# soedinglab/BaMMmotif2

Hardware: AMD Instinct MI355X
Metric: EM seq-positions/sec (and iterations/sec), 1Mx200bp k=2 W=20 (higher is better)
Workload: dtype f32

## Files before the change

### bammmotif2_amd/__init__.py

```python
from . import abi, synth
from .em import (EM, Comm, Context, PackedSeqs, SeqSet, calculate_p, logodds, occurrences, Occurrences, FdrMops, fdr_geometry, seed_from_pwm, sample_negatives, libc_srand,
                 v_size, v_offset, bg_size, bg_offset, device_count, device_pci_bus_id, device_can_access_peer, peer_access_matrix, device_blocks_live, mask_plan)

__all__ = ["EM", "Comm", "Context", "PackedSeqs", "SeqSet", "calculate_p", "logodds", "occurrences", "Occurrences", "FdrMops", "fdr_geometry", "seed_from_pwm", "sample_negatives", "libc_srand",
           "v_size", "v_offset", "bg_size", "bg_offset", "device_count", "device_pci_bus_id", "device_can_access_peer", "peer_access_matrix", "device_blocks_live", "mask_plan", "abi", "synth"]
```

### bammmotif2_amd/abi.py

```python
from __future__ import annotations

import ctypes as C
import os

import numpy as np

HERE = os.path.dirname(os.path.abspath(__file__))
LIB_PATH = os.path.join(HERE, "libbamm_em.so")

OK, ERR_ARG, ERR_HIP, ERR_NO_DEVICE, ERR_UNSUPPORTED, ERR_STATE, ERR_COMM = 0, -1, -2, -3, -4, -5, -6
MAX_ORDER = 10


class BammError(RuntimeError):
    def __init__(self, code: int, msg: str):
        super().__init__(f"bamm error {code}: {msg}")
        self.code = code


class Packed(C.Structure):
    _fields_ = [("n_seqs", C.c_uint64), ("n_words", C.c_uint64), ("n_exc", C.c_uint64),
                ("total_len", C.c_uint64), ("max_len", C.c_uint32), ("min_len", C.c_uint32),
                ("words", C.POINTER(C.c_uint32)), ("word_off", C.POINTER(C.c_uint64)),
                ("len", C.POINTER(C.c_uint32)), ("exc_off", C.POINTER(C.c_uint64)),
# ... 7 lines not shown
                ("n_seqs_global", C.c_uint64), ("n_seqs_bound", C.c_uint64)]


ALLREDUCE_FN = C.CFUNCTYPE(C.c_int, C.c_void_p, C.c_void_p, C.c_uint64, C.c_void_p)

SYMBOLS = [
    "bamm_last_error", "bamm_version", "bamm_pack_kmers", "bamm_pack_kmer_ptrs", "bamm_pack_codes", "bamm_pack_codes_seeded",
    "bamm_unpack_y", "bamm_packed_free", "bamm_shard_range", "bamm_ctx_create", "bamm_ctx_destroy",
    "bamm_ctx_sync", "bamm_ctx_device_name", "bamm_ctx_set_launch", "bamm_ctx_set_tuning", "bamm_seqs_upload",
    "bamm_seqs_destroy", "bamm_seqs_info", "bamm_em_default_params", "bamm_em_create",
    "bamm_em_destroy", "bamm_em_estep", "bamm_em_mstep", "bamm_em_optimize_q", "bamm_em_iterate",
    "bamm_em_optimize", "bamm_em_mask", "bamm_em_accumulate", "bamm_em_reduce_buffer", "bamm_em_update", "bamm_em_set_reduce_buffer",
    "bamm_em_set_allreduce", "bamm_em_set_comm", "bamm_comm_init_all", "bamm_comm_unique_id", "bamm_comm_init_rank",
    "bamm_comm_info", "bamm_comm_destroy", "bamm_comm_time_allreduce", "bamm_em_comm_mode", "bamm_seqs_from_codes", "bamm_seqs_bg_model", "bamm_sample_negatives", "bamm_rand_stream_draws", "bamm_comm_init_local", "bamm_comm_init_shm", "bamm_comm_abort", "bamm_device_count", "bamm_device_pci_bus_id", "bamm_device_can_access_peer", "bamm_em_get_v", "bamm_em_get_counts", "bamm_em_get_s", "bamm_em_get_q",
    "bamm_em_get_llh", "bamm_em_get_vdiff", "bamm_em_get_iteration", "bamm_em_get_r",
    "bamm_em_get_trace", "bamm_em_kernel_time", "bamm_em_set_kernel_timing", "bamm_em_plan", "bamm_em_plan_mixed", "bamm_em_plan_paths", "bamm_mask_plan", "bamm_device_blocks_live", "bamm_seed_from_pwm", "bamm_set_host_threads", "bamm_logodds", "bamm_logodds_subset", "bamm_occurrences", "bamm_occ_info", "bamm_occ_get", "bamm_occ_destroy", "bamm_em_sites", "bamm_sites_info", "bamm_sites_get", "bamm_sites_best", "bamm_sites_destroy", "bamm_fdr_create", "bamm_fdr_add_set", "bamm_fdr_add_scores", "bamm_fdr_seal", "bamm_fdr_absorb", "bamm_fdr_statistics", "bamm_fdr_info", "bamm_fdr_rows", "bamm_fdr_pvalues", "bamm_fdr_geometry", "bamm_fdr_destroy", "bamm_bg_model", "bamm_calculate_p", "bamm_v_size",
    "bamm_v_offset", "bamm_bg_size",
]

_lib = None


def load() -> C.CDLL:
    global _lib
    if _lib is not None:
        return _lib
    if not os.path.exists(LIB_PATH):
        raise ImportError(
            f"{LIB_PATH} is missing: build it with `python -m bammmotif2_amd.build` "
            "(hipcc --offload-arch=gfx950). There is no CPU fallback.")
    L = C.CDLL(LIB_PATH)
# ... 53 lines not shown
    L.bamm_device_pci_bus_id.argtypes = [i, C.c_char_p, C.c_size_t]
    L.bamm_device_can_access_peer.argtypes = [i, i, P(i)]
    for name in ("bamm_em_get_v", "bamm_em_get_counts", "bamm_em_get_s"):
        getattr(L, name).argtypes = [vp, f32p]
    for name in ("bamm_em_get_q", "bamm_em_get_llh", "bamm_em_get_vdiff"):
        getattr(L, name).argtypes = [vp, P(f)]
    L.bamm_em_get_iteration.argtypes = [vp, P(u32)]
    L.bamm_em_get_r.argtypes = [vp, u64, u64, f32p, u64]
    L.bamm_em_get_trace.argtypes = [vp, f32p, f32p, f32p, u32, P(u32)]
    L.bamm_em_kernel_time.argtypes = [vp, P(f), P(u32)]
    L.bamm_em_set_kernel_timing.argtypes = [vp, u32]
    L.bamm_em_plan.argtypes = [vp, P(u64), P(u64), P(u32)]
    L.bamm_em_plan_mixed.argtypes = [vp, P(u64)]
    L.bamm_em_plan_paths.argtypes = [vp, P(i), P(i), P(u64)]
    L.bamm_mask_plan.argtypes = [u32, u32, u32, u64, u64, i, u64p]
    L.bamm_device_blocks_live.argtypes = []
    L.bamm_device_blocks_live.restype = C.c_longlong
    L.bamm_set_host_threads.argtypes = [u32]
    L.bamm_set_host_threads.restype = None
    L.bamm_seed_from_pwm.argtypes = [vp, vp, u32, u32, f32p, f, vp, vp, vp]
    L.bamm_logodds.argtypes = [vp, vp, u32, u32, u32, f32p, f32p, vp, u64, f32p, u64p]
    L.bamm_logodds_subset.argtypes = [vp, vp, vp, u32, u32, u32, f32p, f32p, vp, u64, f32p, u64p]
    L.bamm_occurrences.argtypes = [vp, vp, vp, u32, u32, u32, f32p, f32p, f, P(vp)]
    L.bamm_occ_info.argtypes = [vp, P(u64), P(u64), P(u32), P(f), P(f), P(u64)]
    L.bamm_occ_get.argtypes = [vp, vp, vp, vp, vp, vp, vp, u64]
    L.bamm_occ_destroy.argtypes = [vp]
    L.bamm_em_sites.argtypes = [vp, u64, u64, f, P(vp)]
    L.bamm_sites_info.argtypes = [vp, P(u64), P(u64)]
    L.bamm_sites_get.argtypes = [vp, vp, vp, vp, u64]
    L.bamm_sites_best.argtypes = [vp, vp, vp, vp, u64]
# ... 27 lines not shown
```

### bammmotif2_amd/csrc/common.h

```cpp
#pragma once
#include <hip/hip_runtime.h>

#include <cstdint>
#include <cstdio>
#include <cstring>
#include <map>
#include <memory>
#include <string>
#include <vector>

#include "../../include/bamm_em.h"

namespace bamm {

void set_error(const char* fmt, ...);

#define BAMM_HIP(expr)                                                                        \
    do {                                                                                      \
        hipError_t e_ = (expr);                                                               \
        if (e_ != hipSuccess) {                                                               \
            ::bamm::set_error("%s failed: %s (%s:%d)", #expr, hipGetErrorString(e_), __FILE__, \
                              __LINE__);                                                      \
            return BAMM_ERR_HIP;                                                              \
        }                                                                                     \
// ... 161 lines not shown
    UpdateArgs upd;
    PeerArgs peer;
};

bool grp_geometry(uint32_t K, uint32_t W, uint32_t G, int M, uint32_t waves, bool accum, uint32_t logC, uint32_t layout,
                  GrpGeom* out);
bool grp_plan(uint32_t K, uint32_t W, int M, uint32_t waves, bool many_exceptions, bool enough_work, uint32_t forced_G,
              int forced_layout, uint32_t* G, uint32_t* logC, uint32_t* layout);
bool grp_supported_class(int M, uint32_t K);
int launch_em_grp_long(int mclass, bool accum, bool write_r, const GrpKernelArgs& a, uint32_t blocks, uint32_t threads,
                       hipStream_t st);
int launch_em_grp_xl(int mclass, bool accum, bool write_r, const GrpKernelArgs& a, uint32_t blocks, uint32_t threads,
                     hipStream_t st);
uint32_t grp_max_threads(int M);
bool mix_geometry(uint32_t K, uint32_t W, int M, uint32_t waves, bool accum, GrpGeom* out);
int launch_em_mix(int mclass, bool accum, bool write_r, const GrpKernelArgs& a, uint32_t blocks, uint32_t threads, hipStream_t st);
int launch_em_mix1(int mclass, bool accum, bool write_r, const GrpKernelArgs& a, uint32_t blocks, uint32_t threads, hipStream_t st);
int launch_em_grp(int mclass, bool accum, bool write_r, const GrpKernelArgs& a, uint32_t blocks, uint32_t threads,
                  hipStream_t st);
int launch_mix_records(int mclass, const SeqView& sv, const uint4* xrec, uint32_t W, uint32_t T, uint32_t B, uint2* out,
                       uint32_t num_cus, hipStream_t st);

struct SeedKernelArgs {
    SeqView  sv;
    uint32_t K, W, Y;
    uint32_t max_len, vsize;
    uint32_t table_bytes, count_bytes, wave_bytes;
    const float* score;
    float    q;
    const double* u;
    int*     counts;
    uint32_t* z_out;
    unsigned char* wave_scratch;
};
size_t seed_global_scratch_bytes(const SeedKernelArgs& a, uint32_t num_cus);
// ... 161 lines not shown
```

### bammmotif2_amd/csrc/lane_records.h

```cpp
#pragma once
#include "grouped_kernel.h"

namespace bamm {
namespace {

constexpr uint32_t kMixBj = 6u, kMixNe = 3u, kMixBv = kMixBj + kMixNe;
constexpr uint32_t kMixFixBit = 1u << 31;

template <int M>
__device__ __forceinline__ uint2 mix_lane_record(const RawSeqG<M>& cur, int lane, uint32_t W, uint32_t T, uint32_t B) {
    constexpr uint32_t Y = 64u;
    const uint32_t L = __builtin_amdgcn_readfirstlane(cur.L);
    const uint32_t LW1 = L - W + 1u;
    const uint32_t p0 = (uint32_t)lane * M;

    uint32_t X, sE;
    {
        constexpr int NSEL = RawSeqG<M>::NSEL;
        const uint32_t wi0 = p0 >> 4;
        const uint32_t pE = LW1 - 1u, lpE = pE / (uint32_t)M;
        const uint32_t pe = p0 + (uint32_t)(M - 1);
        const uint32_t sel = (pe >> 4) - wi0;
        uint32_t lo = cur.w[1], hi = cur.w[0];
#pragma unroll
        for (int c = 1; c < NSEL; c++) {
            lo = (sel == (uint32_t)c) ? cur.w[c + 1] : lo;
            hi = (sel == (uint32_t)c) ? cur.w[c] : hi;
        }
        X = __builtin_amdgcn_alignbit(hi, lo, 30u - 2u * (pe & 15u));
        sE = (uint32_t)__builtin_amdgcn_readlane((int)X, (int)lpE) >> (2u * ((uint32_t)(M - 1) - (pE - lpE * (uint32_t)M)));
    }

    const uint32_t lane_b = (uint32_t)lane / T, lane_t = (uint32_t)lane - lane_b * T;
    const uint32_t lane_G = lane_t >= B ? 4u : 3u;
    const uint32_t xw = __builtin_amdgcn_readfirstlane(cur.xr.x);
    const uint32_t Bx = (xw >> 12) & 0xfu;
    const uint32_t xlo = xw & 0xfffu;
    const uint32_t nE = min(kMixNe, L - LW1);
    uint32_t yfix = Y | (Y << 7) | (Y << 14) | (Y << 21);
    const bool fixJ = lane_b < Bx;
    const bool fixE = lane_b >= kMixBj && lane_b < kMixBj + nE;
    if (fixJ || fixE) {
        const uint32_t pv = fixJ ? xlo + lane_b : LW1 + (lane_b - kMixBj);
        const uint32_t xfields = xrec_fields<7>(cur.xr.y, cur.xr.z, cur.xr.w, lane_b + 4u - lane_G);
#pragma unroll
        for (int c = 0; c < 4; c++) {
            uint32_t yc = Y;
            if ((uint32_t)c < lane_G) {
                const uint32_t pos = pv - (lane_G - 1u) + (uint32_t)c;
                if (fixJ) {
                    yc = (xfields >> (7u * (uint32_t)c)) & 0x7fu;
                } else {
                    yc = (sE >> (2u * ((LW1 - 1u - pos) & 15u))) & (Y - 1u);
                }
                if (pos >= LW1) yc = Y;
            }
            yfix = (yfix & ~(0x7fu << (7 * c))) | (yc << (7 * c));
        }
        yfix |= kMixFixBit;
    }
    return make_uint2(X, yfix);
}

struct MixSeq {
    uint32_t seq, L, xw;
    uint2 rec;
    bool ok;
};

__device__ __forceinline__ MixSeq fetch_mix_seq(const SeqView& sv, const uint4* xrec, const uint2* lane_rec, uint32_t t, int lane) {
    MixSeq r;
    r.rec = lane_rec[(size_t)t * 64u + (uint32_t)lane];
    r.seq = pick_sequence(sv, t);
    r.ok = !(sv.mask && !sv.mask[r.seq]);
    r.L = sv.len[r.seq];
// ... 7 lines not shown
```

### bammmotif2_amd/csrc/lane_records.hip

```cpp
#include <algorithm>

#include "lane_records.h"

namespace bamm {
namespace {

constexpr uint32_t kRecThreads = 256u, kRecWaves = kRecThreads / 64u;

template <int M>
__global__ void __launch_bounds__(kRecThreads) k_mix_records(SeqView sv, const uint4* xrec, uint32_t W, uint32_t T, uint32_t B, uint2* out) {
    const int lane = threadIdx.x & 63;
    const uint32_t total_waves = gridDim.x * kRecWaves;
    for (uint32_t t = blockIdx.x * kRecWaves + (threadIdx.x >> 6); t < sv.count; t += total_waves) {
        const RawSeqG<M> cur = fetch_seq_g<M>(sv, xrec, t, lane);
        out[(size_t)t * 64u + (uint32_t)lane] = mix_lane_record<M>(cur, lane, W, T, B);
    }
}

template <int M>
int launch_records(const SeqView& sv, const uint4* xrec, uint32_t W, uint32_t T, uint32_t B, uint2* out, uint32_t blocks, hipStream_t st) {
    return launch_kernel(&k_mix_records<M>, blocks, kRecThreads, 0, st, sv, xrec, W, T, B, out);
}

}

int launch_mix_records(int mclass, const SeqView& sv, const uint4* xrec, uint32_t W, uint32_t T, uint32_t B, uint2* out,
                       uint32_t num_cus, hipStream_t st) {
    if (sv.count == 0u && num_cus != kPrimeOnly) return BAMM_OK;
    const uint32_t blocks = num_cus == kPrimeOnly ? kPrimeOnly
                                                  : std::min((sv.count + kRecWaves - 1u) / kRecWaves, std::max(1u, num_cus) * 8u);
    int rc = BAMM_ERR_UNSUPPORTED;
    switch (mclass) {
        case 3: rc = launch_records<4>(sv, xrec, W, T, B, out, blocks, st); break;
        case 4: rc = launch_records<5>(sv, xrec, W, T, B, out, blocks, st); break;
        case 5: rc = launch_records<6>(sv, xrec, W, T, B, out, blocks, st); break;
        case 6: rc = launch_records<7>(sv, xrec, W, T, B, out, blocks, st); break;
        case 7: rc = launch_records<8>(sv, xrec, W, T, B, out, blocks, st); break;
        case 8: rc = launch_records<10>(sv, xrec, W, T, B, out, blocks, st); break;
        default: set_error("no mixed-row kernel for M class %d", mclass);
    }
    if (rc) return rc;
    if (blocks != kPrimeOnly) BAMM_HIP(hipGetLastError());
    return BAMM_OK;
}

}
```

### bammmotif2_amd/csrc/mixed_kernel.h

```cpp
#pragma once
#include "lane_records.h"

namespace bamm {
namespace {

template <int OFF>
__device__ __forceinline__ void lds_add_u64_exec_big(uint32_t byte_addr, unsigned long long v, unsigned long long mask) {
    static_assert(OFF >= 0 && OFF < 65536, "ds offset field");
    lds_add_u64_exec<OFF>(byte_addr, v, mask);
}

template <int M, int A, int NQ, bool ACCUM, bool WRITE_R, int THREADS>
__global__ void __launch_bounds__(THREADS) k_em_mix(GrpKernelArgs ga) {
    static_assert(M >= 4 && 2 * (M - 1) + 12 <= 32, "a wide group within one lane's run, rows out of one stream window");
    static_assert(A == 1 || A == 2, "wide groups");
    constexpr uint32_t WAVES = THREADS / 64, V = WAVES * kMixBv;
    constexpr uint32_t R5N = 1024u, R5V0 = R5N + 1u, R5T = R5V0 + V;
    constexpr uint32_t R6N = 4096u, R6V0 = R6N + 1u, R6T = R6V0 + V;
    constexpr uint32_t Y = 64u, Ys = 65u;
    if (ga.e.stop != nullptr && *ga.e.stop != 0u) return;
    extern __shared__ __align__(16) unsigned char lds_raw[];
    BAMM_PHASE(0);
    const EmKernelArgs& a = ga.e;
    const GrpGeom& g = ga.g;
    const uint32_t W = a.W, T = g.T, B = g.mixB;
    const uint32_t pad = 4u * NQ - B;
    const uint32_t rs5 = g.rowstride;
    float* sg5 = reinterpret_cast<float*>(lds_raw + g.off_sg);
    float* sg6 = reinterpret_cast<float*>(lds_raw + g.off_sg6);
    const float* s1_stage = reinterpret_cast<const float*>(lds_raw + g.off_s1);
    double* stat_lds = reinterpret_cast<double*>(lds_raw + g.off_stat);
    unsigned long long* cnt5 = reinterpret_cast<unsigned long long*>(lds_raw + g.off_ng);
    unsigned long long* cnt6 = reinterpret_cast<unsigned long long*>(lds_raw + g.off_ng6);
    unsigned long long* n1 = reinterpret_cast<unsigned long long*>(lds_raw + g.off_n1);
    unsigned long long* n1p = reinterpret_cast<unsigned long long*>(lds_raw + g.off_wave);
    const uint32_t n1c = ACCUM ? g.wave_bytes / (Y * 8u) : 0u;

    const int lane = threadIdx.x & 63;
    const uint32_t wave = __builtin_amdgcn_readfirstlane(threadIdx.x >> 6);
    const uint32_t total_waves = gridDim.x * WAVES;
    uint32_t t = blockIdx.x * WAVES + wave;
    MixSeq nxt{};
    if (t < a.sv.count) nxt = fetch_mix_seq(a.sv, ga.xrec, ga.lane_rec, t, lane);

    [[maybe_unused]] float q_fused = 0.0f;
    {
        float* s1w = reinterpret_cast<float*>(lds_raw + g.off_s1);
        const float* s1 = s1_stage;
        bool staged = false;
        if constexpr (ACCUM) {
            if (ga.fused) {
// ... 42 lines not shown
            __syncthreads();
        }
    }

    BAMM_PHASE(2);
    if constexpr (ACCUM) {
        const __attribute__((address_space(4))) GrpKernelArgs* kq =
            (const __attribute__((address_space(4))) GrpKernelArgs*)__builtin_amdgcn_kernarg_segment_ptr();
        asm volatile("" : "+s"(kq));
        if (kq->peer.world > 1u && *kq->peer.err != 0u) return;
    }
    const float q = (ACCUM && ga.fused) ? q_fused : *a.q;
    const float one_minus_q = 1.0f - q;
    const uint32_t lane_b = (uint32_t)lane / T, lane_t = (uint32_t)lane - lane_b * T;
    const bool lane_wide = lane_t >= B;
    const uint32_t lane_col0 = lane_wide ? 3u * B + 4u * (lane_t - B) : 3u * lane_t;
    const uint32_t vbase5 = R5V0 + wave * kMixBv, vbase6 = R6V0 + wave * kMixBv;
    const uint32_t sg5_base = lds_offset(sg5), sg6_base = lds_offset(sg6);

    uint32_t resident_fill = 0u;
#pragma unroll
    for (int c = 0; c < 4; c++)
        if (lane_col0 + (uint32_t)c < n1c) resident_fill |= Y << (7 * c);
    double llh_acc = 0.0, sumr_acc = 0.0;
    uint32_t seq_cnt = 0, last_LW1 = 0;
    float pos_i = 0.0f;
    float pos_m[M];
    constexpr bool kCacheSpec = M <= 7 || THREADS < 1024;
    [[maybe_unused]] int spec[kCacheSpec ? M : 1];
    [[maybe_unused]] uint32_t spec_LW1 = 0, spec_xw = 0xffffffffu;
#pragma unroll
    for (int m = 0; m < M; m++) pos_m[m] = 0.0f;
#pragma unroll
    for (int m = 0; m < (kCacheSpec ? M : 1); m++) spec[m] = -1;
    [[maybe_unused]] GrpLogEntry* my_log = nullptr;
    [[maybe_unused]] uint32_t nlog = 0;
    if constexpr (ACCUM)
        my_log = reinterpret_cast<GrpLogEntry*>(ga.fix_log) + (size_t)(blockIdx.x * WAVES + wave) * ga.fix_log_cap;

    for (; t < a.sv.count; t += total_waves) {
        const MixSeq cur = nxt;
        const __attribute__((address_space(4))) GrpKernelArgs* kp =
            (const __attribute__((address_space(4))) GrpKernelArgs*)__builtin_amdgcn_kernarg_segment_ptr();
        asm volatile("" : "+s"(kp));
        if (t + total_waves < a.sv.count) {
            SeqView sv2;
            sv2.words = nullptr; sv2.word_off = nullptr; sv2.len = kp->e.sv.len; sv2.pos_off = nullptr;
            sv2.exc_off = nullptr; sv2.exc = nullptr; sv2.mask = kp->e.sv.mask; sv2.idx = kp->e.sv.idx; sv2.count = a.sv.count;
            nxt = fetch_mix_seq(sv2, kp->xrec, kp->lane_rec, t + total_waves, lane);
        }
        const uint32_t seq = cur.seq;
        if (WRITE_R && (seq < a.seq_begin || seq >= a.seq_end)) continue;
        if (!cur.ok) continue;
        __builtin_amdgcn_s_setprio(0);
        const uint32_t L = __builtin_amdgcn_readfirstlane(cur.L);
        const uint32_t LW1 = L - W + 1u;
        const uint32_t p0 = (uint32_t)lane * M;

        const uint32_t X = cur.rec.x, yfix = cur.rec.y;
        const bool fix = (int)yfix < 0;
        const uint32_t xw = __builtin_amdgcn_readfirstlane(cur.xw);
        const uint32_t Bx = (xw >> 12) & 0xfu;
        const uint32_t xlo = xw & 0xfffu;
        const uint32_t nE = min(kMixNe, L - LW1);
        float fs[4] = {1.0f, 1.0f, 1.0f, 1.0f};
        const float* const sfix_now = (ACCUM && kp->fused) ? kp->s_block + (size_t)blockIdx.x * (W * Ys) : kp->e.s;
        if (fix) {
#pragma unroll
            for (int c = 0; c < 4; c++) {
                const uint32_t colc = min(lane_col0 + (uint32_t)c, W - 1u);
                fs[c] = sfix_now[__umul24(colc, Ys) + ((yfix >> (7 * c)) & 0x7fu)];
            }
        }
        auto slot_offsets = [&](int (&o)[M]) {
#pragma unroll
            for (int m = 0; m < M; m++) {
                const uint32_t k2 = p0 + m - xlo, k3 = p0 + m - LW1;
                o[m] = (p0 + m < LW1) ? -1 : 0;
                if (k2 < Bx) o[m] = (int)(1u + wave * kMixBv + k2);
                if (k3 < nE) o[m] = (int)(1u + wave * kMixBv + kMixBj + k3);
            }
        };
        uint32_t row5[M], row6[M];
        if constexpr (kCacheSpec) {
            if (LW1 != spec_LW1 || xw != spec_xw) {
                spec_LW1 = LW1; spec_xw = xw;
                slot_offsets(spec);
            }
#pragma unroll
            for (int m = 0; m < M; m++) {
                const bool stream = spec[m] < 0;
                row5[m] = stream ? ((X >> (2 * (M - 1 - m))) & 1023u) : R5N + (uint32_t)spec[m];
                row6[m] = stream ? ((X >> (2 * (M - 1 - m))) & 4095u) : R6N + (uint32_t)spec[m];
            }
        } else {
            int o[M];
            slot_offsets(o);
#pragma unroll
            for (int m = 0; m < M; m++) {
                const bool stream = o[m] < 0;
                row5[m] = stream ? ((X >> (2 * (M - 1 - m))) & 1023u) : R5N + (uint32_t)o[m];
                row6[m] = stream ? ((X >> (2 * (M - 1 - m))) & 4095u) : R6N + (uint32_t)o[m];
            }
        }
        if (fix) {
            const float f = ((fs[0] * fs[1]) * fs[2]) * fs[3];
            if (lane_wide) sg6[(vbase6 + lane_b) * A + (lane_t - B)] = f;
            else sg5[__umul24(vbase5 + lane_b, rs5) + pad + lane_t] = f;
        }
        wave_lds_sync();

        __builtin_amdgcn_s_setprio(2);
        float U[M];
        {
            uint32_t ra[M];
#pragma unroll
            for (int m = 0; m < M; m++) ra[m] = sg5_base + __umul24(row5[m], rs5 * 4u);
            float2 pr[M];
#pragma unroll
            for (int m = 0; m < M; m++) {
#ifdef BAMM_PLAIN_LDS
                if constexpr (A == 2) pr[m] = lds_load<float2>(sg6_base + row6[m] * 8u);
                else pr[m].x = lds_load<float>(sg6_base + row6[m] * 4u);
#else
                if constexpr (A == 2) asm volatile("ds_read_b64 %0, %1" : "=v"(pr[m]) : "v"(sg6_base + row6[m] * 8u));
                else asm volatile("ds_read_b32 %0, %1" : "=v"(pr[m].x) : "v"(sg6_base + row6[m] * 4u));
#endif
            }
            grp_chain<M, 3, NQ>(ra, U);
            lds_wait(pr);
            float w0[M];
#pragma unroll
// ... 39 lines not shown
                const uint32_t p = p0 + m;
                if (p < L) ro[L - 1u - p] = U[m];
            }
        }

        if (ACCUM) {
            __builtin_amdgcn_s_setprio(3);
            unsigned long long F[M], nz[M];
            uint32_t rad6[M], rad5[M];
            const uint32_t c5 = lds_offset(cnt5), c6 = lds_offset(cnt6);
#pragma unroll
            for (int m = 0; m < M; m++) {
                F[m] = to_fixed40_pre(U[m]);
                nz[m] = __ballot(F[m] != 0ull);
                rad6[m] = c6 + row6[m] * 8u;
                rad5[m] = c5 + row5[m] * 8u;
            }
            static_for<A>([&](auto wc) {
                constexpr int w = decltype(wc)::value;
                constexpr int off = (4 * w) % M;
#pragma unroll
                for (int m = 0; m < M; m++)
                    lds_add_u64_exec_big<(int)(w * R6T * 8u)>(rad6[m], F[(m + off) % M], nz[(m + off) % M]);
#pragma unroll
                for (int c = 0; c < 4; c++) {
                    const int idx = (c + off) % M;
                    F[idx] = wave_shl1_u64(F[idx]);
                    nz[idx] >>= 1;
                }
            });
            static_for<4 * NQ>([&](auto uc) {
// ... 7 lines not shown
                    for (int c = 0; c < 3; c++) {
                        const int idx = (c + off) % M;
                        F[idx] = wave_shl1_u64(F[idx]);
                        nz[idx] >>= 1;
                    }
                }
            });
            wave_lds_sync();
            unsigned long long acc = 0ull;
            if (fix) {
                unsigned long long* cell = lane_wide ? cnt6 + (size_t)(T - 1u - lane_t) * R6T + vbase6 + lane_b
                                                     : cnt5 + (size_t)(B - 1u - lane_t) * R5T + vbase5 + lane_b;
                acc = *cell;
                *cell = 0ull;
            }
            if (acc != 0ull) {
#pragma unroll
                for (int c = 0; c < 4; c++) {
                    const uint32_t yc = (yfix >> (7 * c)) & 0x7fu;
                    if (yc < Y && ((resident_fill >> (7 * c + 6)) & 1u) != 0u)
                        atomicAdd(&n1p[(lane_col0 + (uint32_t)c) * Y + yc], acc);
                }
            }
            const uint32_t ylog = yfix | resident_fill;
            const uint32_t code = lane_t | (ylog << 3);
            if ((~ylog & (Y | (Y << 7) | (Y << 14) | (Y << 21))) == 0u) acc = 0ull;
            const unsigned long long nzm = __ballot(acc != 0ull);
            if (acc != 0ull) {
                const uint32_t rank = __builtin_amdgcn_mbcnt_hi((uint32_t)(nzm >> 32), __builtin_amdgcn_mbcnt_lo((uint32_t)nzm, 0u));
                GrpLogEntry* const log_now = reinterpret_cast<GrpLogEntry*>(kp->fix_log) + (size_t)(blockIdx.x * WAVES + wave) * kp->fix_log_cap;
                grp_log_store(log_now, nlog + rank, acc, code);
            }
            nlog += (uint32_t)__builtin_popcountll(nzm);
            wave_lds_sync();
        }
    }

    lds_drain();
    BAMM_PHASE(3);
    __syncthreads();
    BAMM_PHASE(4);
    if (lane == 0) {
        stat_lds[wave * 3 + 0] = llh_acc;
// ... 131 lines not shown
```

### bammmotif2_amd/csrc/plan.cpp

```cpp

#include <atomic>
#include <cmath>

#include "handles.h"

namespace bamm {

namespace {

constexpr size_t kLds = 160 * 1024;

int prime_bucket(bamm_ctx* c, const bamm_em_params& prm, uint32_t Y, bool sliced, const EmBucket& eb) {
    if (hipSetDevice(c->device) != hipSuccess) { set_error("hipSetDevice failed"); return BAMM_ERR_HIP; }
    EmKernelArgs a{};
    a.K = prm.K; a.W = prm.W; a.Y = Y;
    if (eb.mclass == kLongClass) return launch_long_em(a, true, false, false, kPrimeOnly, c->stream);
    const uint32_t threads = bucket_threads(c, eb);
    if (sliced || !eb.grouped) {
        a.logC = 0;
        return launch_em_seq(eb.mclass, false, false, a, kPrimeOnly, threads, c->stream);
    }
    GrpKernelArgs ga{};
    ga.e = a;
    if (!grp_geometry(prm.K, prm.W, eb.G, kMClasses[eb.mclass], threads / 64u, true, eb.logc, eb.layout, &ga.g)) return BAMM_OK;
    if (eb.layout & 8u)
        if (int rc = launch_mix_records(eb.mclass, SeqView{}, nullptr, prm.W, ga.g.T, ga.g.mixB, nullptr, kPrimeOnly, c->stream)) return rc;
    return launch_em_grp(eb.mclass, true, false, ga, kPrimeOnly, threads, c->stream);
}

}

uint32_t default_threads(const bamm_ctx* c, int mclass) {
    uint32_t t = c->threads ? c->threads : max_threads_for_mclass(mclass);
    return std::min(t, max_threads_for_mclass(mclass));
}

uint32_t bucket_threads(const bamm_ctx* c, const EmBucket& b) {
    if (b.mclass == kLongClass) return 256u;
    const uint32_t t = default_threads(c, b.mclass);
    return b.grouped ? std::min(t, grp_max_threads(kMClasses[b.mclass])) : t;
}
// ... 103 lines not shown
                    (capable(n) ? yes : no).push_back(n);
                }
            EmBucket eb;
            eb.mclass = b.mclass; eb.grouped = true; eb.logc = glogc; eb.G = gG; eb.layout = glayout; eb.d_xrec = xr->d_xrec;
            if (all) { eb.count = b.count; eb.d_idx = b.d_idx; }
            else {
                uint32_t* d = nullptr;
                if ((rc = em->mem.upload(&d, yes.data(), yes.size()))) return rc;
                own_lists = true;
                eb.count = (uint32_t)yes.size(); eb.d_idx = d;
            }
            if ((glayout & 8u) && eb.count) {
                uint2* rec = nullptr;
                if ((rc = em->mem.scratch(&rec, (size_t)eb.count * 64u))) return rc;
                if ((rc = launch_mix_records(eb.mclass, make_view(seqs, em->exc, eb.d_idx, eb.count, nullptr), xr->d_xrec, prm->W,
                                             gg.T, gg.mixB, rec, (uint32_t)std::max(1, c->num_cus), st))) return rc;
                eb.d_lane_rec = rec;
            }
            eb.work = (double)eb.count * Mcls * 0.6;
            if (eb.count) em->ebuckets.push_back(eb);
            if (all) continue;
        }
        EmBucket eb;
        eb.mclass = b.mclass;
        if (!no.empty()) {
            uint32_t* d = nullptr;
            if ((rc = em->mem.upload(&d, no.data(), no.size()))) return rc;
            own_lists = true;
            eb.count = (uint32_t)no.size(); eb.d_idx = d;
        } else { eb.count = b.count; eb.d_idx = b.d_idx; }
        eb.work = (double)eb.count * Mcls;
// ... 116 lines not shown
```

### bammmotif2_amd/em.py

```python
from __future__ import annotations

import ctypes as C
from typing import Callable, Optional

import numpy as np

from . import abi
from .abi import check


def _f32(a):
    return np.ascontiguousarray(a, dtype=np.float32)


def _u64(a):
    return np.ascontiguousarray(a, dtype=np.uint64)


def v_size(K: int, W: int) -> int:
    return W * ((4 ** (K + 2) - 4) // 3)


def v_offset(k: int, W: int) -> int:
    return W * ((4 ** (k + 1) - 4) // 3)
# ... 110 lines not shown
    return int(n.value)


def device_blocks_live() -> int:
    return int(abi.load().bamm_device_blocks_live())


MASK_PLAN_FIELDS = ("direct", "wave_global", "wave_bytes", "s_in_lds", "e_table", "m_cols", "m_table", "init_table", "e_waves",
                    "m_waves", "cus", "mblocks", "wave_scratch_bytes")


def mask_plan(W: int, Y: int, max_len: int, n_seqs: int, cells: int, num_cus: int) -> dict:
    out = np.zeros(len(MASK_PLAN_FIELDS), np.uint64)
    check(abi.load().bamm_mask_plan(W, Y, max_len, n_seqs, cells, num_cus, out))
    return dict(zip(MASK_PLAN_FIELDS, (int(x) for x in out)))


def device_pci_bus_id(device: int) -> str:
    buf = C.create_string_buffer(32)
    check(abi.load().bamm_device_pci_bus_id(int(device), buf, 32))
    return buf.value.decode()


def device_can_access_peer(device: int, peer: int) -> bool:
    can = C.c_int(0)
    check(abi.load().bamm_device_can_access_peer(int(device), int(peer), C.byref(can)))
    return bool(can.value)


def peer_access_matrix():
# ... 478 lines not shown
```

### include/bamm_em.h

```cpp
#ifndef BAMM_EM_H_
#define BAMM_EM_H_

#include <stddef.h>
#include <stdint.h>

#ifdef __cplusplus
extern "C" {
#endif

#define BAMM_OK              0
#define BAMM_ERR_ARG        -1
#define BAMM_ERR_HIP        -2
#define BAMM_ERR_NO_DEVICE  -3
#define BAMM_ERR_UNSUPPORTED -4
#define BAMM_ERR_STATE      -5
#define BAMM_ERR_COMM       -6

#define BAMM_MAX_ORDER      10
#define BAMM_MAX_SEQ_POSITIONS 8192u

typedef struct bamm_ctx  bamm_ctx;
typedef struct bamm_seqs bamm_seqs;
typedef struct bamm_em   bamm_em;
typedef struct bamm_comm bamm_comm;
// ... 108 lines not shown
typedef struct bamm_sites bamm_sites;
int  bamm_em_sites(bamm_em* em, uint64_t begin, uint64_t end, float cutoff, bamm_sites** out);
int  bamm_sites_info(const bamm_sites* s, uint64_t* n_sites, uint64_t* n_seqs);
int  bamm_sites_get(const bamm_sites* s, uint64_t* seq, uint32_t* pos, float* r, uint64_t cap);
int  bamm_sites_best(const bamm_sites* s, uint32_t* z, float* r_best, uint32_t* count, uint64_t cap);
int  bamm_sites_destroy(bamm_sites* s);
int  bamm_em_get_trace(bamm_em* em, float* llh, float* v_diff, float* q, uint32_t cap, uint32_t* n);
#define BAMM_TIMING_WHOLE_CALL 0xffffffffu
int  bamm_em_kernel_time(bamm_em* em, float* total_ms, uint32_t* launches);
int  bamm_em_set_kernel_timing(bamm_em* em, uint32_t every);
int  bamm_em_plan(bamm_em* em, uint64_t* grouped_seqs, uint64_t* percolumn_seqs, uint32_t* launches);
int  bamm_em_plan_mixed(bamm_em* em, uint64_t* mixed_seqs);
int  bamm_em_plan_paths(bamm_em* em, int* sliced, int* e_fused, uint64_t* long_seqs);
int  bamm_mask_plan(uint32_t W, uint32_t Y, uint32_t max_len, uint64_t n_seqs, uint64_t cells, int num_cus, uint64_t* out);

int  bamm_seed_from_pwm(bamm_ctx* ctx, bamm_seqs* seqs, uint32_t K, uint32_t W, const float* score,
                        float q, const double* u, int32_t* counts, uint32_t* z);

int  bamm_logodds(bamm_ctx* ctx, bamm_seqs* seqs, uint32_t K, uint32_t W, uint32_t bg_order,
                  const float* v_flat, const float* vbg, float* mops, uint64_t mops_cap,
                  float* zoops, uint64_t* z);

int  bamm_logodds_subset(bamm_ctx* ctx, bamm_seqs* seqs, const uint8_t* seq_mask, uint32_t K, uint32_t W,
                         uint32_t bg_order, const float* v_flat, const float* vbg, float* mops,
                         uint64_t mops_cap, float* zoops, uint64_t* z);

typedef struct bamm_occ bamm_occ;
int  bamm_occurrences(bamm_ctx* ctx, bamm_seqs* positives, bamm_seqs* negatives, uint32_t K, uint32_t W,
                      uint32_t bg_order, const float* v_flat, const float* vbg, float p_cutoff, bamm_occ** out);
int  bamm_occ_info(const bamm_occ* occ, uint64_t* n_hits, uint64_t* n_neg_scores, uint32_t* n_top, float* s_ntop,
// ... 38 lines not shown
```

Measured before the change: 501.9 billion.

## Precompute mixed-row fix-lane log decision and simplify inner-loop row/address math

Moves the per-lane decision of whether a fix lane must log to the global fix log into the precomputed lane record, stored as a bit in the yfix word, and encodes the fix flag in bit 31 of the window word. In the mixed E-step kernel it replaces the per-sequence resident-fill loop and atomics with precomputed ballot masks and exec-masked LDS adds. It also biases row5 offsets so row5/row6 come from a max() instead of selects, and hoists fix addresses. This trims scalar/vector ALU work in the hot loop, at the cost of more subtle encoding invariants. Host-callable test hooks are added for the layout and fix word.

```diff
diff --git a/bammmotif2_amd/__init__.py b/bammmotif2_amd/__init__.py
--- a/bammmotif2_amd/__init__.py
+++ b/bammmotif2_amd/__init__.py
@@ -1,6 +1,6 @@
 from . import abi, synth
 from .em import (EM, Comm, Context, PackedSeqs, SeqSet, calculate_p, logodds, occurrences, Occurrences, FdrMops, fdr_geometry, seed_from_pwm, sample_negatives, libc_srand,
-                 v_size, v_offset, bg_size, bg_offset, device_count, device_pci_bus_id, device_can_access_peer, peer_access_matrix, device_blocks_live, mask_plan)
+                 v_size, v_offset, bg_size, bg_offset, device_count, device_pci_bus_id, device_can_access_peer, peer_access_matrix, device_blocks_live, mask_plan, mix_layout, mix_fix_word)
 
 __all__ = ["EM", "Comm", "Context", "PackedSeqs", "SeqSet", "calculate_p", "logodds", "occurrences", "Occurrences", "FdrMops", "fdr_geometry", "seed_from_pwm", "sample_negatives", "libc_srand",
-           "v_size", "v_offset", "bg_size", "bg_offset", "device_count", "device_pci_bus_id", "device_can_access_peer", "peer_access_matrix", "device_blocks_live", "mask_plan", "abi", "synth"]
+           "v_size", "v_offset", "bg_size", "bg_offset", "device_count", "device_pci_bus_id", "device_can_access_peer", "peer_access_matrix", "device_blocks_live", "mask_plan", "mix_layout", "mix_fix_word", "abi", "synth"]
diff --git a/bammmotif2_amd/abi.py b/bammmotif2_amd/abi.py
--- a/bammmotif2_amd/abi.py
+++ b/bammmotif2_amd/abi.py
@@ -45,7 +45,7 @@
     "bamm_em_set_allreduce", "bamm_em_set_comm", "bamm_comm_init_all", "bamm_comm_unique_id", "bamm_comm_init_rank",
     "bamm_comm_info", "bamm_comm_destroy", "bamm_comm_time_allreduce", "bamm_em_comm_mode", "bamm_seqs_from_codes", "bamm_seqs_bg_model", "bamm_sample_negatives", "bamm_rand_stream_draws", "bamm_comm_init_local", "bamm_comm_init_shm", "bamm_comm_abort", "bamm_device_count", "bamm_device_pci_bus_id", "bamm_device_can_access_peer", "bamm_em_get_v", "bamm_em_get_counts", "bamm_em_get_s", "bamm_em_get_q",
     "bamm_em_get_llh", "bamm_em_get_vdiff", "bamm_em_get_iteration", "bamm_em_get_r",
-    "bamm_em_get_trace", "bamm_em_kernel_time", "bamm_em_set_kernel_timing", "bamm_em_plan", "bamm_em_plan_mixed", "bamm_em_plan_paths", "bamm_mask_plan", "bamm_device_blocks_live", "bamm_seed_from_pwm", "bamm_set_host_threads", "bamm_logodds", "bamm_logodds_subset", "bamm_occurrences", "bamm_occ_info", "bamm_occ_get", "bamm_occ_destroy", "bamm_em_sites", "bamm_sites_info", "bamm_sites_get", "bamm_sites_best", "bamm_sites_destroy", "bamm_fdr_create", "bamm_fdr_add_set", "bamm_fdr_add_scores", "bamm_fdr_seal", "bamm_fdr_absorb", "bamm_fdr_statistics", "bamm_fdr_info", "bamm_fdr_rows", "bamm_fdr_pvalues", "bamm_fdr_geometry", "bamm_fdr_destroy", "bamm_bg_model", "bamm_calculate_p", "bamm_v_size",
+    "bamm_em_get_trace", "bamm_em_kernel_time", "bamm_em_set_kernel_timing", "bamm_em_plan", "bamm_em_plan_mixed", "bamm_em_plan_paths", "bamm_mask_plan", "bamm_mix_layout", "bamm_mix_fix_word", "bamm_device_blocks_live", "bamm_seed_from_pwm", "bamm_set_host_threads", "bamm_logodds", "bamm_logodds_subset", "bamm_occurrences", "bamm_occ_info", "bamm_occ_get", "bamm_occ_destroy", "bamm_em_sites", "bamm_sites_info", "bamm_sites_get", "bamm_sites_best", "bamm_sites_destroy", "bamm_fdr_create", "bamm_fdr_add_set", "bamm_fdr_add_scores", "bamm_fdr_seal", "bamm_fdr_absorb", "bamm_fdr_statistics", "bamm_fdr_info", "bamm_fdr_rows", "bamm_fdr_pvalues", "bamm_fdr_geometry", "bamm_fdr_destroy", "bamm_bg_model", "bamm_calculate_p", "bamm_v_size",
     "bamm_v_offset", "bamm_bg_size",
 ]
 
@@ -129,6 +129,8 @@
     L.bamm_em_plan_mixed.argtypes = [vp, P(u64)]
     L.bamm_em_plan_paths.argtypes = [vp, P(i), P(i), P(u64)]
     L.bamm_mask_plan.argtypes = [u32, u32, u32, u64, u64, i, u64p]
+    L.bamm_mix_layout.argtypes = [u32, i, P(u32)]
+    L.bamm_mix_fix_word.argtypes = [u32, u32, u32, u32, u32, u32, u32, u32, u32, P(u32)]
     L.bamm_device_blocks_live.argtypes = []
     L.bamm_device_blocks_live.restype = C.c_longlong
     L.bamm_set_host_threads.argtypes = [u32]
diff --git a/bammmotif2_amd/csrc/common.h b/bammmotif2_amd/csrc/common.h
--- a/bammmotif2_amd/csrc/common.h
+++ b/bammmotif2_amd/csrc/common.h
@@ -199,11 +199,12 @@
                      hipStream_t st);
 uint32_t grp_max_threads(int M);
 bool mix_geometry(uint32_t K, uint32_t W, int M, uint32_t waves, bool accum, GrpGeom* out);
+inline __host__ __device__ uint32_t mix_resident_cols(const GrpGeom& g) { return g.wave_bytes / (64u * 8u); }
 int launch_em_mix(int mclass, bool accum, bool write_r, const GrpKernelArgs& a, uint32_t blocks, uint32_t threads, hipStream_t st);
 int launch_em_mix1(int mclass, bool accum, bool write_r, const GrpKernelArgs& a, uint32_t blocks, uint32_t threads, hipStream_t st);
 int launch_em_grp(int mclass, bool accum, bool write_r, const GrpKernelArgs& a, uint32_t blocks, uint32_t threads,
                   hipStream_t st);
-int launch_mix_records(int mclass, const SeqView& sv, const uint4* xrec, uint32_t W, uint32_t T, uint32_t B, uint2* out,
+int launch_mix_records(int mclass, const SeqView& sv, const uint4* xrec, uint32_t W, uint32_t T, uint32_t B, uint32_t n1c, uint2* out,
                        uint32_t num_cus, hipStream_t st);
 
 struct SeedKernelArgs {
diff --git a/bammmotif2_amd/csrc/lane_records.h b/bammmotif2_amd/csrc/lane_records.h
--- a/bammmotif2_amd/csrc/lane_records.h
+++ b/bammmotif2_amd/csrc/lane_records.h
@@ -6,10 +6,53 @@
 
 constexpr uint32_t kMixBj = 6u, kMixNe = 3u, kMixBv = kMixBj + kMixNe;
 constexpr uint32_t kMixFixBit = 1u << 31;
+constexpr uint32_t kMixLogBit = 1u << 31;
+constexpr uint32_t kMixNoY = 64u | (64u << 7) | (64u << 14) | (64u << 21);
+
+__host__ __device__ inline uint32_t mix_resident_fill(uint32_t lane_col0, uint32_t n1c) {
+    uint32_t fill = 0u;
+    for (uint32_t c = 0; c < 4u; c++)
+        if (lane_col0 + c < n1c) fill |= 64u << (7u * c);
+    return fill;
+}
+
+__host__ __device__ inline uint32_t mix_group_col0(uint32_t t, uint32_t B) { return t >= B ? 3u * B + 4u * (t - B) : 3u * t; }
+
+__host__ __device__ inline uint32_t mix_fix_word(uint32_t lane, uint32_t W, uint32_t T, uint32_t B, uint32_t n1c, uint32_t L, uint32_t xw,
+                                                 uint32_t xfields, uint32_t sE, bool* fix) {
+    constexpr uint32_t Y = 64u;
+    const uint32_t LW1 = L - W + 1u;
+    const uint32_t lane_b = lane / T, lane_t = lane - lane_b * T;
+    const uint32_t lane_G = lane_t >= B ? 4u : 3u;
+    const uint32_t Bx = (xw >> 12) & 0xfu;
+    const uint32_t xlo = xw & 0xfffu;
+    const uint32_t nE = L - LW1 < kMixNe ? L - LW1 : kMixNe;
+    uint32_t yfix = kMixNoY;
+    const bool fixJ = lane_b < Bx;
+    const bool fixE = lane_b >= kMixBj && lane_b < kMixBj + nE;
+    *fix = fixJ || fixE;
+    if (!*fix) return yfix;
+    const uint32_t pv = fixJ ? xlo + lane_b : LW1 + (lane_b - kMixBj);
+    for (uint32_t c = 0; c < 4u; c++) {
+        uint32_t yc = Y;
+        if (c < lane_G) {
+            const uint32_t pos = pv - (lane_G - 1u) + c;
+            if (fixJ) {
+                yc = (xfields >> (7u * c)) & 0x7fu;
+            } else {
+                yc = (sE >> (2u * ((LW1 - 1u - pos) & 15u))) & (Y - 1u);
+            }
+            if (pos >= LW1) yc = Y;
+        }
+        yfix = (yfix & ~(0x7fu << (7u * c))) | (yc << (7u * c));
+    }
+    if ((~(yfix | mix_resident_fill(mix_group_col0(lane_t, B), n1c)) & kMixNoY) != 0u) yfix |= kMixLogBit;
+    return yfix;
+}
 
 template <int M>
-__device__ __forceinline__ uint2 mix_lane_record(const RawSeqG<M>& cur, int lane, uint32_t W, uint32_t T, uint32_t B) {
-    constexpr uint32_t Y = 64u;
+__device__ __forceinline__ uint2 mix_lane_record(const RawSeqG<M>& cur, int lane, uint32_t W, uint32_t T, uint32_t B, uint32_t n1c) {
+    static_assert(2 * (M - 1) + 12 <= 31, "bit 31 of the window word is the fix-lane flag");
     const uint32_t L = __builtin_amdgcn_readfirstlane(cur.L);
     const uint32_t LW1 = L - W + 1u;
     const uint32_t p0 = (uint32_t)lane * M;
@@ -31,34 +74,13 @@
         sE = (uint32_t)__builtin_amdgcn_readlane((int)X, (int)lpE) >> (2u * ((uint32_t)(M - 1) - (pE - lpE * (uint32_t)M)));
     }
 
+    const uint32_t xw = __builtin_amdgcn_readfirstlane(cur.xr.x);
     const uint32_t lane_b = (uint32_t)lane / T, lane_t = (uint32_t)lane - lane_b * T;
     const uint32_t lane_G = lane_t >= B ? 4u : 3u;
-    const uint32_t xw = __builtin_amdgcn_readfirstlane(cur.xr.x);
-    const uint32_t Bx = (xw >> 12) & 0xfu;
-    const uint32_t xlo = xw & 0xfffu;
-    const uint32_t nE = min(kMixNe, L - LW1);
-    uint32_t yfix = Y | (Y << 7) | (Y << 14) | (Y << 21);
-    const bool fixJ = lane_b < Bx;
-    const bool fixE = lane_b >= kMixBj && lane_b < kMixBj + nE;
-    if (fixJ || fixE) {
-        const uint32_t pv = fixJ ? xlo + lane_b : LW1 + (lane_b - kMixBj);
-        const uint32_t xfields = xrec_fields<7>(cur.xr.y, cur.xr.z, cur.xr.w, lane_b + 4u - lane_G);
-#pragma unroll
-        for (int c = 0; c < 4; c++) {
-            uint32_t yc = Y;
-            if ((uint32_t)c < lane_G) {
-                const uint32_t pos = pv - (lane_G - 1u) + (uint32_t)c;
-                if (fixJ) {
-                    yc = (xfields >> (7u * (uint32_t)c)) & 0x7fu;
-                } else {
-                    yc = (sE >> (2u * ((LW1 - 1u - pos) & 15u))) & (Y - 1u);
-                }
-                if (pos >= LW1) yc = Y;
-            }
-            yfix = (yfix & ~(0x7fu << (7 * c))) | (yc << (7 * c));
-        }
-        yfix |= kMixFixBit;
-    }
+    const uint32_t xfields = xrec_fields<7>(cur.xr.y, cur.xr.z, cur.xr.w, lane_b + 4u - lane_G);
+    bool fix;
+    const uint32_t yfix = mix_fix_word((uint32_t)lane, W, T, B, n1c, L, xw, xfields, sE, &fix);
+    X = (X & ~kMixFixBit) | (fix ? kMixFixBit : 0u);
     return make_uint2(X, yfix);
 }
 
diff --git a/bammmotif2_amd/csrc/lane_records.hip b/bammmotif2_amd/csrc/lane_records.hip
--- a/bammmotif2_amd/csrc/lane_records.hip
+++ b/bammmotif2_amd/csrc/lane_records.hip
@@ -8,35 +8,35 @@
 constexpr uint32_t kRecThreads = 256u, kRecWaves = kRecThreads / 64u;
 
 template <int M>
-__global__ void __launch_bounds__(kRecThreads) k_mix_records(SeqView sv, const uint4* xrec, uint32_t W, uint32_t T, uint32_t B, uint2* out) {
+__global__ void __launch_bounds__(kRecThreads) k_mix_records(SeqView sv, const uint4* xrec, uint32_t W, uint32_t T, uint32_t B, uint32_t n1c, uint2* out) {
     const int lane = threadIdx.x & 63;
     const uint32_t total_waves = gridDim.x * kRecWaves;
     for (uint32_t t = blockIdx.x * kRecWaves + (threadIdx.x >> 6); t < sv.count; t += total_waves) {
         const RawSeqG<M> cur = fetch_seq_g<M>(sv, xrec, t, lane);
-        out[(size_t)t * 64u + (uint32_t)lane] = mix_lane_record<M>(cur, lane, W, T, B);
+        out[(size_t)t * 64u + (uint32_t)lane] = mix_lane_record<M>(cur, lane, W, T, B, n1c);
     }
 }
 
 template <int M>
-int launch_records(const SeqView& sv, const uint4* xrec, uint32_t W, uint32_t T, uint32_t B, uint2* out, uint32_t blocks, hipStream_t st) {
-    return launch_kernel(&k_mix_records<M>, blocks, kRecThreads, 0, st, sv, xrec, W, T, B, out);
+int launch_records(const SeqView& sv, const uint4* xrec, uint32_t W, uint32_t T, uint32_t B, uint32_t n1c, uint2* out, uint32_t blocks, hipStream_t st) {
+    return launch_kernel(&k_mix_records<M>, blocks, kRecThreads, 0, st, sv, xrec, W, T, B, n1c, out);
 }
 
 }
 
-int launch_mix_records(int mclass, const SeqView& sv, const uint4* xrec, uint32_t W, uint32_t T, uint32_t B, uint2* out,
+int launch_mix_records(int mclass, const SeqView& sv, const uint4* xrec, uint32_t W, uint32_t T, uint32_t B, uint32_t n1c, uint2* out,
                        uint32_t num_cus, hipStream_t st) {
     if (sv.count == 0u && num_cus != kPrimeOnly) return BAMM_OK;
     const uint32_t blocks = num_cus == kPrimeOnly ? kPrimeOnly
                                                   : std::min((sv.count + kRecWaves - 1u) / kRecWaves, std::max(1u, num_cus) * 8u);
     int rc = BAMM_ERR_UNSUPPORTED;
     switch (mclass) {
-        case 3: rc = launch_records<4>(sv, xrec, W, T, B, out, blocks, st); break;
-        case 4: rc = launch_records<5>(sv, xrec, W, T, B, out, blocks, st); break;
-        case 5: rc = launch_records<6>(sv, xrec, W, T, B, out, blocks, st); break;
-        case 6: rc = launch_records<7>(sv, xrec, W, T, B, out, blocks, st); break;
-        case 7: rc = launch_records<8>(sv, xrec, W, T, B, out, blocks, st); break;
-        case 8: rc = launch_records<10>(sv, xrec, W, T, B, out, blocks, st); break;
+        case 3: rc = launch_records<4>(sv, xrec, W, T, B, n1c, out, blocks, st); break;
+        case 4: rc = launch_records<5>(sv, xrec, W, T, B, n1c, out, blocks, st); break;
+        case 5: rc = launch_records<6>(sv, xrec, W, T, B, n1c, out, blocks, st); break;
+        case 6: rc = launch_records<7>(sv, xrec, W, T, B, n1c, out, blocks, st); break;
+        case 7: rc = launch_records<8>(sv, xrec, W, T, B, n1c, out, blocks, st); break;
+        case 8: rc = launch_records<10>(sv, xrec, W, T, B, n1c, out, blocks, st); break;
         default: set_error("no mixed-row kernel for M class %d", mclass);
     }
     if (rc) return rc;
@@ -45,3 +45,23 @@
 }
 
 }
+
+extern "C" int bamm_mix_layout(uint32_t W, int M, uint32_t* out) {
+    bamm::GrpGeom g{};
+    if (!out) { bamm::set_error("bamm_mix_layout: bad argument"); return BAMM_ERR_ARG; }
+    if (M < 1 || !bamm::mix_geometry(2u, W, M, bamm::grp_max_threads(M) / 64u, true, &g)) {
+        bamm::set_error("no mixed rows for W=%u at %d positions per lane", W, M);
+        return BAMM_ERR_UNSUPPORTED;
+    }
+    out[0] = g.T; out[1] = g.mixB; out[2] = g.mixA; out[3] = bamm::mix_resident_cols(g);
+    return BAMM_OK;
+}
+
+extern "C" int bamm_mix_fix_word(uint32_t lane, uint32_t W, uint32_t T, uint32_t B, uint32_t n1c, uint32_t L, uint32_t xw, uint32_t xfields,
+                                 uint32_t sE, uint32_t* out) {
+    if (!out || lane >= 64u || !T || B > T || W > L) { bamm::set_error("bamm_mix_fix_word: bad argument"); return BAMM_ERR_ARG; }
+    bool fix = false;
+    out[0] = bamm::mix_fix_word(lane, W, T, B, n1c, L, xw, xfields, sE, &fix);
+    out[1] = fix ? 1u : 0u;
+    return BAMM_OK;
+}
diff --git a/bammmotif2_amd/csrc/mixed_kernel.h b/bammmotif2_amd/csrc/mixed_kernel.h
--- a/bammmotif2_amd/csrc/mixed_kernel.h
+++ b/bammmotif2_amd/csrc/mixed_kernel.h
@@ -3,6 +3,19 @@
 
 namespace bamm {
 namespace {
+
+__device__ __forceinline__ uint32_t field7(uint32_t w, int at) {
+    uint32_t f;
+    asm("v_bfe_u32 %0, %1, %2, 7" : "=v"(f) : "v"(w), "n"(at));
+    return f;
+}
+
+constexpr uint32_t kMixRow5Bias = 3072u;
+__device__ __forceinline__ void mix_rows(uint32_t X, int at, uint32_t special, uint32_t& row5_biased, uint32_t& row6) {
+    const uint32_t six = (X >> at) & 4095u;
+    row6 = max(six, special);
+    row5_biased = max(six | kMixRow5Bias, special);
+}
 
 template <int OFF>
 __device__ __forceinline__ void lds_add_u64_exec_big(uint32_t byte_addr, unsigned long long v, unsigned long long mask) {
@@ -34,7 +47,7 @@
     unsigned long long* cnt6 = reinterpret_cast<unsigned long long*>(lds_raw + g.off_ng6);
     unsigned long long* n1 = reinterpret_cast<unsigned long long*>(lds_raw + g.off_n1);
     unsigned long long* n1p = reinterpret_cast<unsigned long long*>(lds_raw + g.off_wave);
-    const uint32_t n1c = ACCUM ? g.wave_bytes / (Y * 8u) : 0u;
+    const uint32_t n1c = ACCUM ? mix_resident_cols(g) : 0u;
 
     const int lane = threadIdx.x & 63;
     const uint32_t wave = __builtin_amdgcn_readfirstlane(threadIdx.x >> 6);
@@ -107,14 +120,24 @@
     const float one_minus_q = 1.0f - q;
     const uint32_t lane_b = (uint32_t)lane / T, lane_t = (uint32_t)lane - lane_b * T;
     const bool lane_wide = lane_t >= B;
-    const uint32_t lane_col0 = lane_wide ? 3u * B + 4u * (lane_t - B) : 3u * lane_t;
+    const uint32_t lane_col0 = mix_group_col0(lane_t, B);
     const uint32_t vbase5 = R5V0 + wave * kMixBv, vbase6 = R6V0 + wave * kMixBv;
-    const uint32_t sg5_base = lds_offset(sg5), sg6_base = lds_offset(sg6);
-
-    uint32_t resident_fill = 0u;
-#pragma unroll
-    for (int c = 0; c < 4; c++)
-        if (lane_col0 + (uint32_t)c < n1c) resident_fill |= Y << (7 * c);
+    const uint32_t sg6_base = lds_offset(sg6);
+    const uint32_t sg5_base_biased = lds_offset(sg5) - kMixRow5Bias * (rs5 * 4u);
+
+    const uint32_t resident_fill = mix_resident_fill(lane_col0, n1c);
+    [[maybe_unused]] uint32_t code_fill = lane_t | (resident_fill << 3);
+    asm volatile("" : "+v"(code_fill));
+    [[maybe_unused]] const bool resident_wide = __builtin_amdgcn_readfirstlane((uint32_t)(n1c > 3u * B + 3u)) != 0u;
+    [[maybe_unused]] unsigned long long resident_lanes[4];
+#pragma unroll
+    for (int c = 0; c < 4; c++) {
+        resident_lanes[c] = __builtin_amdgcn_ballot_w64(((resident_fill >> (7 * c + 6)) & 1u) != 0u);
+        asm volatile("" : "+s"(resident_lanes[c]));
+    }
+    const uint32_t fix_s1 = __umul24(lane_col0, Ys * 4u);
+    float* const fix_odds = lane_wide ? sg6 + ((vbase6 + lane_b) * A + (lane_t - B)) : sg5 + (__umul24(vbase5 + lane_b, rs5) + pad + lane_t);
+    [[maybe_unused]] const uint32_t fix_bin = lds_offset(n1p) + lane_col0 * (Y * 8u);
     double llh_acc = 0.0, sumr_acc = 0.0;
     uint32_t seq_cnt = 0, last_LW1 = 0;
     float pos_i = 0.0f;
@@ -125,7 +148,7 @@
 #pragma unroll
     for (int m = 0; m < M; m++) pos_m[m] = 0.0f;
 #pragma unroll
-    for (int m = 0; m < (kCacheSpec ? M : 1); m++) spec[m] = -1;
+    for (int m = 0; m < (kCacheSpec ? M : 1); m++) spec[m] = 0;
     [[maybe_unused]] GrpLogEntry* my_log = nullptr;
     [[maybe_unused]] uint32_t nlog = 0;
     if constexpr (ACCUM)
@@ -151,29 +174,31 @@
         const uint32_t p0 = (uint32_t)lane * M;
 
         const uint32_t X = cur.rec.x, yfix = cur.rec.y;
-        const bool fix = (int)yfix < 0;
+        const bool fix = (int)X < 0;
         const uint32_t xw = __builtin_amdgcn_readfirstlane(cur.xw);
         const uint32_t Bx = (xw >> 12) & 0xfu;
         const uint32_t xlo = xw & 0xfffu;
         const uint32_t nE = min(kMixNe, L - LW1);
-        float fs[4] = {1.0f, 1.0f, 1.0f, 1.0f};
-        const float* const sfix_now = (ACCUM && kp->fused) ? kp->s_block + (size_t)blockIdx.x * (W * Ys) : kp->e.s;
+        float fs[4];
+        uint32_t yf[4];
+#pragma unroll
+        for (int c = 0; c < 4; c++) yf[c] = field7(yfix, 7 * c);
+        const char* const sfix_now = reinterpret_cast<const char*>((ACCUM && kp->fused) ? kp->s_block + (size_t)blockIdx.x * (W * Ys) : kp->e.s);
         if (fix) {
 #pragma unroll
-            for (int c = 0; c < 4; c++) {
-                const uint32_t colc = min(lane_col0 + (uint32_t)c, W - 1u);
-                fs[c] = sfix_now[__umul24(colc, Ys) + ((yfix >> (7 * c)) & 0x7fu)];
-            }
+            for (int c = 0; c < 4; c++)
+                fs[c] = *reinterpret_cast<const float*>(sfix_now + ((yf[c] << 2) + fix_s1) + c * (int)(Ys * 4u));
         }
         auto slot_offsets = [&](int (&o)[M]) {
 #pragma unroll
             for (int m = 0; m < M; m++) {
                 const uint32_t k2 = p0 + m - xlo, k3 = p0 + m - LW1;
-                o[m] = (p0 + m < LW1) ? -1 : 0;
-                if (k2 < Bx) o[m] = (int)(1u + wave * kMixBv + k2);
-                if (k3 < nE) o[m] = (int)(1u + wave * kMixBv + kMixBj + k3);
+                o[m] = (p0 + m < LW1) ? 0 : (int)R6N;
+                if (k2 < Bx) o[m] = (int)(R6N + 1u + wave * kMixBv + k2);
+                if (k3 < nE) o[m] = (int)(R6N + 1u + wave * kMixBv + kMixBj + k3);
             }
         };
+        static_assert(R6N - R5N == kMixRow5Bias && R5N == 1024u && R6N == 4096u, "mix_rows");
         uint32_t row5[M], row6[M];
         if constexpr (kCacheSpec) {
             if (LW1 != spec_LW1 || xw != spec_xw) {
@@ -181,25 +206,16 @@
                 slot_offsets(spec);
             }
 #pragma unroll
-            for (int m = 0; m < M; m++) {
-                const bool stream = spec[m] < 0;
-                row5[m] = stream ? ((X >> (2 * (M - 1 - m))) & 1023u) : R5N + (uint32_t)spec[m];
-                row6[m] = stream ? ((X >> (2 * (M - 1 - m))) & 4095u) : R6N + (uint32_t)spec[m];
-            }
+            for (int m = 0; m < M; m++) mix_rows(X, 2 * (M - 1 - m), (uint32_t)spec[m], row5[m], row6[m]);
         } else {
             int o[M];
             slot_offsets(o);
 #pragma unroll
-            for (int m = 0; m < M; m++) {
-                const bool stream = o[m] < 0;
-                row5[m] = stream ? ((X >> (2 * (M - 1 - m))) & 1023u) : R5N + (uint32_t)o[m];
-                row6[m] = stream ? ((X >> (2 * (M - 1 - m))) & 4095u) : R6N + (uint32_t)o[m];
-            }
+            for (int m = 0; m < M; m++) mix_rows(X, 2 * (M - 1 - m), (uint32_t)o[m], row5[m], row6[m]);
         }
         if (fix) {
             const float f = ((fs[0] * fs[1]) * fs[2]) * fs[3];
-            if (lane_wide) sg6[(vbase6 + lane_b) * A + (lane_t - B)] = f;
-            else sg5[__umul24(vbase5 + lane_b, rs5) + pad + lane_t] = f;
+            *fix_odds = f;
         }
         wave_lds_sync();
 
@@ -208,7 +224,7 @@
         {
             uint32_t ra[M];
 #pragma unroll
-            for (int m = 0; m < M; m++) ra[m] = sg5_base + __umul24(row5[m], rs5 * 4u);
+            for (int m = 0; m < M; m++) ra[m] = sg5_base_biased + __umul24(row5[m], rs5 * 4u);
             float2 pr[M];
 #pragma unroll
             for (int m = 0; m < M; m++) {
@@ -278,7 +294,7 @@
                 F[m] = to_fixed40_pre(U[m]);
                 nz[m] = __ballot(F[m] != 0ull);
                 rad6[m] = c6 + row6[m] * 8u;
-                rad5[m] = c5 + row5[m] * 8u;
+                rad5[m] = c5 - kMixRow5Bias * 8u + row5[m] * 8u;
             }
             static_for<A>([&](auto wc) {
                 constexpr int w = decltype(wc)::value;
@@ -316,19 +332,16 @@
                 acc = *cell;
                 *cell = 0ull;
             }
-            if (acc != 0ull) {
-#pragma unroll
-                for (int c = 0; c < 4; c++) {
-                    const uint32_t yc = (yfix >> (7 * c)) & 0x7fu;
-                    if (yc < Y && ((resident_fill >> (7 * c + 6)) & 1u) != 0u)
-                        atomicAdd(&n1p[(lane_col0 + (uint32_t)c) * Y + yc], acc);
-                }
-            }
-            const uint32_t ylog = yfix | resident_fill;
-            const uint32_t code = lane_t | (ylog << 3);
-            if ((~ylog & (Y | (Y << 7) | (Y << 14) | (Y << 21))) == 0u) acc = 0ull;
-            const unsigned long long nzm = __ballot(acc != 0ull);
-            if (acc != 0ull) {
+            const unsigned long long has_acc = __builtin_amdgcn_ballot_w64(acc != 0ull);
+            static_for<4>([&](auto cc) {
+                constexpr int c = decltype(cc)::value;
+                if (c == 3 && !resident_wide) return;
+                lds_add_u64_exec<c * (int)(Y * 8u)>(fix_bin + (yf[c] << 3), acc, has_acc & resident_lanes[c] & __builtin_amdgcn_ballot_w64(yf[c] < Y));
+            });
+            const uint32_t code = code_fill | (yfix << 3);
+            const bool to_log = acc != 0ull && (int)yfix < 0;
+            const unsigned long long nzm = has_acc & __builtin_amdgcn_ballot_w64((int)yfix < 0);
+            if (to_log) {
                 const uint32_t rank = __builtin_amdgcn_mbcnt_hi((uint32_t)(nzm >> 32), __builtin_amdgcn_mbcnt_lo((uint32_t)nzm, 0u));
                 GrpLogEntry* const log_now = reinterpret_cast<GrpLogEntry*>(kp->fix_log) + (size_t)(blockIdx.x * WAVES + wave) * kp->fix_log_cap;
                 grp_log_store(log_now, nlog + rank, acc, code);
diff --git a/bammmotif2_amd/csrc/plan.cpp b/bammmotif2_amd/csrc/plan.cpp
--- a/bammmotif2_amd/csrc/plan.cpp
+++ b/bammmotif2_amd/csrc/plan.cpp
@@ -24,7 +24,7 @@
     ga.e = a;
     if (!grp_geometry(prm.K, prm.W, eb.G, kMClasses[eb.mclass], threads / 64u, true, eb.logc, eb.layout, &ga.g)) return BAMM_OK;
     if (eb.layout & 8u)
-        if (int rc = launch_mix_records(eb.mclass, SeqView{}, nullptr, prm.W, ga.g.T, ga.g.mixB, nullptr, kPrimeOnly, c->stream)) return rc;
+        if (int rc = launch_mix_records(eb.mclass, SeqView{}, nullptr, prm.W, ga.g.T, ga.g.mixB, 0u, nullptr, kPrimeOnly, c->stream)) return rc;
     return launch_em_grp(eb.mclass, true, false, ga, kPrimeOnly, threads, c->stream);
 }
 
@@ -158,7 +158,7 @@
                 uint2* rec = nullptr;
                 if ((rc = em->mem.scratch(&rec, (size_t)eb.count * 64u))) return rc;
                 if ((rc = launch_mix_records(eb.mclass, make_view(seqs, em->exc, eb.d_idx, eb.count, nullptr), xr->d_xrec, prm->W,
-                                             gg.T, gg.mixB, rec, (uint32_t)std::max(1, c->num_cus), st))) return rc;
+                                             gg.T, gg.mixB, mix_resident_cols(gg), rec, (uint32_t)std::max(1, c->num_cus), st))) return rc;
                 eb.d_lane_rec = rec;
             }
             eb.work = (double)eb.count * Mcls * 0.6;
diff --git a/bammmotif2_amd/em.py b/bammmotif2_amd/em.py
--- a/bammmotif2_amd/em.py
+++ b/bammmotif2_amd/em.py
@@ -148,6 +148,18 @@
     out = np.zeros(len(MASK_PLAN_FIELDS), np.uint64)
     check(abi.load().bamm_mask_plan(W, Y, max_len, n_seqs, cells, num_cus, out))
     return dict(zip(MASK_PLAN_FIELDS, (int(x) for x in out)))
+
+
+def mix_layout(W: int, M: int) -> dict:
+    out = (C.c_uint32 * 4)()
+    check(abi.load().bamm_mix_layout(W, M, out))
+    return dict(zip(("T", "B", "A", "n1c"), (int(x) for x in out)))
+
+
+def mix_fix_word(lane: int, W: int, T: int, B: int, n1c: int, L: int, xw: int, xfields: int, sE: int):
+    out = (C.c_uint32 * 2)()
+    check(abi.load().bamm_mix_fix_word(lane, W, T, B, n1c, L, xw, xfields, sE, out))
+    return int(out[0]), bool(out[1])
 
 
 def device_pci_bus_id(device: int) -> str:
diff --git a/include/bamm_em.h b/include/bamm_em.h
--- a/include/bamm_em.h
+++ b/include/bamm_em.h
@@ -146,6 +146,10 @@
 int  bamm_em_plan_paths(bamm_em* em, int* sliced, int* e_fused, uint64_t* long_seqs);
 int  bamm_mask_plan(uint32_t W, uint32_t Y, uint32_t max_len, uint64_t n_seqs, uint64_t cells, int num_cus, uint64_t* out);
 
+int  bamm_mix_layout(uint32_t W, int M, uint32_t* out);
+int  bamm_mix_fix_word(uint32_t lane, uint32_t W, uint32_t T, uint32_t B, uint32_t n1c, uint32_t L, uint32_t xw, uint32_t xfields,
+                       uint32_t sE, uint32_t* out);
+
 int  bamm_seed_from_pwm(bamm_ctx* ctx, bamm_seqs* seqs, uint32_t K, uint32_t W, const float* score,
                         float q, const double* u, int32_t* counts, uint32_t* z);
 
```

Measured after the change: 515.5 billion, median of 6. +2.7%, better.
